# sotelo/parrot

Hardware: AMD Instinct MI355X
Metric: acoustic feature frames/sec (train fwd+bwd+allreduce+clip/Adam) (higher is better)
Workload: dtype f32; 1 GPU; BASELINE configs[1]: 2-layer attention-GRU decoder, h=1024, batch=64 per GPU, T_enc=200, T_dec=800, fp32; cell=gru, layers=2, hidden=1024, batch_per_gpu=64, global_batch=64, T_enc=200, T_dec=800, parallelism=dp1, params=13919212

## Files before the change

### include/parrot_hip.h

```cpp
#ifndef PARROT_HIP_H
#define PARROT_HIP_H

#include <stddef.h>
#include <stdint.h>

#ifdef __cplusplus
extern "C" {
#endif

#define PARROT_ERR_BADARG 10001
#define PARROT_ERR_UNSUPPORTED 10002

#define PARROT_NORM_EPS 1e-5f
#define PARROT_MAX_LAYERS 3

const char* parrot_hip_version(void);

int parrot_profile_begin(void);
long long parrot_profile_end(double* total_us, double* flops, double* bytes);
long long parrot_profile_end2(double* total_us, double* flops, double* bytes, double* plain4);

#define PARROT_PRECISION_F32 0
#define PARROT_PRECISION_BF16 1
#define PARROT_PRECISION_BF16X3 2
int parrot_set_gemm_precision(int mode);
int parrot_get_gemm_precision(void);
int parrot_gemm(const float* A, int lda, int transA, const float* B, int ldb, int transB, float* C, int ldc,
                int M, int N, int K, const float* bias, float alpha, int accumulate, int act, int nbatch,
                long long strideA, long long strideB, long long strideC, int split_k, void* stream);

int parrot_gemm_gated(const float* A, int lda, int transA, const float* B, int ldb, int transB, float* C, int ldc,
                      int M, int N, int K, const float* gate, int ldg, void* stream);

#define PARROT_GEMM_ROUTE_STEP 0
#define PARROT_GEMM_ROUTE_F32 1
#define PARROT_GEMM_ROUTE_BF16 2
#define PARROT_GEMM_ROUTE_BF16X3 3
int parrot_gemm_route(const float* A, int lda, int transA, const float* B, int ldb, int transB, int M, int N, int K,
                      float alpha, int act, int nbatch, long long strideA, long long strideB, int split_k, int has_gate,
                      int* kernel, int* slices);

int parrot_step_launch_mode(int njobs, const int* M, const int* N, const int* K, const int* lstm_H, int* info);

int parrot_to_bf16(const float* x, void* y, long long n, void* stream);
int parrot_gemm_bf16in(const void* A, int lda, const void* B, int ldb, float* C, int ldc, int M, int N, int K,
                       int accumulate, int split_k, void* stream);
int parrot_gemm_bf16in_ex(const void* A, int lda, int transA, const void* B, int ldb, int transB, float* C, int ldc, int M,
                          int N, int K, const float* bias, int accumulate, int split_k, void* stream);

int parrot_colsum(const float* x, long long M, int N, int ld, float* out, int accumulate, void* stream);
int parrot_colsum_route(const float* x, long long M, int N, int ld, const float* out, int* info2);

int parrot_gru_step_fwd(const float* h, const float* inputs, const float* gate_inputs, const float* mask,
                        const float* Wg, const float* Wc, float* h_out, float* z, float* r, float* rh,
                        float* c, int B, int H, void* stream);

int parrot_gru_step_bwd(const float* dh_out, const float* h, const float* mask, const float* Wg,
                        const float* Wc, const float* z, const float* r, const float* c, float* dh,
                        float* d_inputs, float* d_gate_inputs, int B, int H, void* stream);

typedef struct ParrotGruSeqDesc {
    int T, B, H, nchain, use_graph, reserved;
    int reverse[4];
    const float* Wg[4];
    const float* Wc[4];
    const float* inputs[4];
    const float* gate_inputs[4];
    const float* mask;
    float* h[4];
    float* z[4]; float* r[4]; float* rh[4]; float* c[4];
    float* dh[4];
    float* dG[4];
    float* dC[4];
// ... 317 lines not shown
```

### parrot_amd/_lib.py

```python
from __future__ import annotations

import ctypes as C
import os

from .utils import env_str

_HERE = os.path.dirname(os.path.abspath(__file__))
LIB_PATH = os.path.join(_HERE, "libparrot_hip.so")

MAX_LAYERS = 3

c_float_p = C.c_void_p


class HipLibraryMissing(RuntimeError):
    pass


class HipCallError(RuntimeError):
    pass


class GruSeqDesc(C.Structure):
    _fields_ = [
# ... 119 lines not shown
        ("eou_extra", C.c_int), ("reserved9", C.c_int),
        ("Wrh_t", C.c_void_p), ("rh_const", C.c_void_p), ("rh_cols", C.c_int), ("reserved10", C.c_int),
        ("Wc_t16", C.c_void_p * MAX_LAYERS),
    ]


class SampleRnnGenDesc(C.Structure):
    _fields_ = ([(n, C.c_int) for n in ("B", "D", "T", "Q", "FS", "BFS", "feat_dim", "use_graph")] +
                [("temperature", C.c_float), ("reserved", C.c_int), ("seed", C.c_ulonglong)] +
                [(n, C.c_void_p) for n in (
                    "big_Win_frames", "big_Win_feats", "big_bin", "big_U", "big_bU", "big_Wg", "big_Wc",
                    "big_Wout", "big_bout", "frm_Win", "frm_bin", "frm_U", "frm_bU", "frm_Wg", "frm_Wc",
                    "frm_Wout", "frm_bout", "emb_tbl", "W2", "b2", "W3", "b3", "W4", "b4", "features",
                    "samples", "big_h", "frm_h", "xf_big", "xf_frm", "feat_cur", "gru_in", "P", "z", "r", "rh",
                    "big_out", "frame_out", "o1", "o2", "o3", "logits", "tbase")] +
                [("n_rnn", C.c_int), ("lstm", C.c_int),
                 ("big_L", (C.c_void_p * 4) * 5), ("frm_L", (C.c_void_p * 4) * 5),
                 ("big_hs", C.c_void_p * 5), ("big_cs", C.c_void_p * 5),
                 ("frm_hs", C.c_void_p * 5), ("frm_cs", C.c_void_p * 5),
                 ("gate_ws", C.c_void_p), ("layer_tmp", C.c_void_p),
                 ("persist_ws", C.c_void_p), ("persist_ws_floats", C.c_longlong)])


_vp, _i, _f, _ll, _sz = C.c_void_p, C.c_int, C.c_float, C.c_longlong, C.c_size_t
SIGNATURES = {
    "parrot_hip_version": (C.c_char_p, []),
    "parrot_profile_begin": (_i, []),
    "parrot_profile_end": (C.c_longlong, [C.POINTER(C.c_double)] * 3),
    "parrot_profile_end2": (C.c_longlong, [C.POINTER(C.c_double)] * 4),
    "parrot_gemm": (_i, [_vp, _i, _i, _vp, _i, _i, _vp, _i, _i, _i, _i, _vp, _f, _i, _i, _i, _ll, _ll, _ll, _i, _vp]),
    "parrot_gemm_gated": (_i, [_vp, _i, _i, _vp, _i, _i, _vp, _i, _i, _i, _i, _vp, _i, _vp]),
    "parrot_gemm_route": (_i, [_vp, _i, _i, _vp, _i, _i, _i, _i, _i, _f, _i, _i, _ll, _ll, _i, _i,
                               C.POINTER(C.c_int), C.POINTER(C.c_int)]),
    "parrot_step_launch_mode": (_i, [_i] + [C.POINTER(C.c_int)] * 5),
    "parrot_gather_sum_fwd": (_i, [_vp, _vp, _vp, _i, _vp, _i, _ll, _i, _i, _i, _vp]),
    "parrot_gather_sum_bwd_ws_floats": (C.c_longlong, [_ll, _i, _i, _i]),
    "parrot_gather_sum_bwd": (_i, [_vp, _i, _vp, _vp, _vp, _vp, _ll, _ll, _i, _i, _i, _i, _vp]),
    "parrot_softmax_ce_fwd": (_i, [_vp, _i, _vp, _ll, _i, _vp, _vp, _vp]),
    "parrot_softmax_ce_bwd": (_i, [_vp, _i, _vp, _vp, _vp, _ll, _i, _vp, _i, _vp]),
    "parrot_relu_gate": (_i, [_vp, _vp, _vp, _ll, _vp]),
    "parrot_gmm_cost_fwd": (_i, [_vp, _i] * 4 + [_ll, _i, _i, _f, _vp, _vp, _i, _vp, _vp]),
    "parrot_gmm_cost_bwd": (_i, [_vp, _i] * 4 + [_vp, _vp, _ll, _i, _i, _f] + [_vp, _i] * 3 + [_vp]),
    "samplernn_weightnorm_ws_floats": (_ll, [_i]),
    "samplernn_weightnorm_fold": (_i, [_vp, _i, _vp, _vp, _i, _vp, _vp, _i, _i, _vp]),
    "samplernn_weightnorm_fold_bwd": (_i, [_vp, _i, _vp, _vp, _vp, _i, _vp, _i, _vp, _vp, _i, _i, _i, _i, _vp]),
    "parrot_colsum": (_i, [_vp, _ll, _i, _i, _vp, _i, _vp]),
    "parrot_colsum_route": (_i, [_vp, _ll, _i, _i, _vp, C.POINTER(C.c_int)]),
    "parrot_gru_step_fwd": (_i, [_vp] * 11 + [_i, _i, _vp]),
    "parrot_gru_step_bwd": (_i, [_vp] * 11 + [_i, _i, _vp]),
    "parrot_label_tables_supported": (_i, [_ll, _i]),
    "parrot_label_gather": (_i, [C.POINTER(LabelTablesDesc), _vp]),
    "parrot_label_segsum_ws_floats": (C.c_longlong, [_ll, _i, _i]),
    "parrot_label_segsum": (_i, [C.POINTER(LabelTablesDesc), _vp, _ll, _vp]),
    "parrot_gru_seq_create": (_i, [C.POINTER(GruSeqDesc), C.POINTER(C.c_void_p)]),
    "parrot_gru_seq_fwd": (_i, [_vp, _vp]),
    "parrot_gru_seq_bwd": (_i, [_vp, _vp]),
    "parrot_gru_seq_destroy": (_i, [_vp]),
    "parrot_gru_seq_route": (_i, [_vp, C.POINTER(C.c_int)]),
    "parrot_gru_seq_rowwise_supported": (_i, [_i, _i, _i, _i]),
    "parrot_lstm_seq_create": (_i, [C.POINTER(LstmSeqDesc), C.POINTER(C.c_void_p)]),
    "parrot_lstm_seq_fwd": (_i, [_vp, _vp]),
    "parrot_lstm_seq_bwd": (_i, [_vp, _vp]),
    "parrot_lstm_seq_destroy": (_i, [_vp]),
    "parrot_gmm_attention_fwd": (_i, [_vp] * 10 + [_i] * 6 + [_f] * 4 + [_vp]),
    "parrot_gmm_attention_bwd": (_i, [_vp] * 10 + [_i] * 6 + [_f, _vp]),
    "parrot_decoder_create": (_i, [C.POINTER(DecoderDesc), C.POINTER(C.c_void_p)]),
# ... 80 lines not shown
```

### parrot_amd/csrc/biggemm.h

```cpp
#pragma once
#include "common.h"

struct BgArgs {
    const float* A;
    const float* B;
    float* C;
    const float* bias;
    int M, N, K;
    long long sam, sak, sbk, sbn;
    int ldc;
    long long batchA, batchB, batchC;
    int nbatch;
    int splitk;
    float* ws;
    int accumulate;
    float alpha;
    int act;
    const float* gate;
    int ldg;
    int bf16;
};

int bg_launch(const BgArgs& a, hipStream_t stream);
void bg_tile_shape(int bf16, int& bm, int& bn);
int bg_to_bf16_launch(const float* x, void* y, long long n, hipStream_t stream);
int bg_reduce_launch(const BgArgs& a, hipStream_t stream);

struct BgPrecisionScope {
    explicit BgPrecisionScope(int bf16);
    ~BgPrecisionScope();
    int saved;
};
```

### parrot_amd/csrc/biggemm.hip

```cpp
#include "biggemm.h"

#include <atomic>

#include <hip/hip_runtime.h>
#include <stdlib.h>
#include <string.h>

namespace {

constexpr int BM = 128, BN = 128, BK = 16, PITCH = 132;

__device__ __forceinline__ void bg_tile_of_block(int bid, int tiles_m, int tiles_n, int& tm, int& tn) {
    const int nwg = tiles_m * tiles_n;
    const int q = nwg / 8, r = nwg % 8;
    const int xcd = bid % 8, idx = bid / 8;
    const int lin = (xcd < r ? xcd * (q + 1) : r * (q + 1) + (xcd - r) * q) + idx;
    constexpr int GW = 8;
    const int group = lin / (GW * tiles_m);
    const int first = group * GW;
    const int gsz = min(tiles_n - first, GW);
    const int rem = lin - group * GW * tiles_m;
    tm = rem / gsz;
    tn = first + rem % gsz;
}

template <bool XC>
__device__ __forceinline__ void bg_load8(const float* __restrict__ p, int x0, int X, int k0, int kend,
                                         long long sx, long long sk, bool vec, int t, f32x4& v) {
    v = (f32x4){0.f, 0.f, 0.f, 0.f};
    if (XC) {
        const int xq = t & 31, kr = t >> 5;
        const int k = k0 + kr, x = x0 + 4 * xq;
        if (k < kend) {
// ... 386 lines not shown
            if (n >= a.N) continue;
            const float bias = (a.bias && ks == 0) ? a.bias[n] : 0.f;
#pragma unroll
            for (int q = 0; q < 16; ++q) {
                const int m = m0 + wm * 128 + i * 32 + (q & 3) + 8 * (q >> 2) + 4 * kk;
                if (m >= a.M) continue;
                const float v = a.alpha * acc[i][j][q];
                if (a.splitk > 1) {
                    a.ws[((long long)z * a.M + m) * a.N + n] = v;
                } else {
                    float* c = C + (long long)m * a.ldc + n;
                    *c = a.accumulate ? *c + v + bias : v + bias;
                }
            }
        }
}

constexpr int SBK = 16;
typedef __bf16 bf16x4 __attribute__((ext_vector_type(4)));

__device__ __forceinline__ void bgs_split(const f32x4& v, bf16x4& p0, bf16x4& p1, bf16x4& p2) {
    p0 = __builtin_convertvector(v, bf16x4);
    const f32x4 r1 = v - __builtin_convertvector(p0, f32x4);
    p1 = __builtin_convertvector(r1, bf16x4);
    const f32x4 r2 = r1 - __builtin_convertvector(p1, f32x4);
    p2 = __builtin_convertvector(r2, bf16x4);
}

template <bool XC>
struct BgsOperand {
    static constexpr int PK = SBK + 8;
    static constexpr int PLANE = XC ? SBK * HPITCH : 256 * PK;
    static constexpr int SZ = 3 * PLANE;
    static __device__ __forceinline__ void load(const float* __restrict__ p, long long ld, int x0, int X, int k0, int kend,
                                                bool vec, int t, f32x4 (&v)[2]) {
#pragma unroll
        for (int i = 0; i < 2; ++i) {
            const int id = t + 512 * i;
            v[i] = (f32x4){0.f, 0.f, 0.f, 0.f};
            if (XC) {
                const int k = k0 + (id >> 6), x = x0 + 4 * (id & 63);
                if (k < kend && x < X) {
                    const float* q = p + (long long)k * ld + x;
                    if (vec && x + 3 < X) v[i] = *reinterpret_cast<const f32x4*>(q);
                    else {
#pragma unroll
                        for (int u = 0; u < 4; ++u)
                            if (x + u < X) v[i][u] = q[u];
                    }
                }
            } else {
                const int x = x0 + (id >> 2), k = k0 + 4 * (id & 3);
                if (x < X && k < kend) {
                    const float* q = p + (long long)x * ld + k;
                    if (vec && k + 3 < kend) v[i] = *reinterpret_cast<const f32x4*>(q);
                    else {
#pragma unroll
                        for (int u = 0; u < 4; ++u)
                            if (k + u < kend) v[i][u] = q[u];
                    }
                }
            }
        }
    }
    static __device__ __forceinline__ void store(__bf16* __restrict__ s, int t, const f32x4 (&v)[2]) {
#pragma unroll
        for (int i = 0; i < 2; ++i) {
            const int id = t + 512 * i;
            bf16x4 p0, p1, p2;
            bgs_split(v[i], p0, p1, p2);
            __bf16* d = XC ? s + (id >> 6) * HPITCH + 4 * (id & 63) : s + (id >> 2) * PK + 4 * (id & 3);
            *reinterpret_cast<bf16x4*>(d) = p0;
            *reinterpret_cast<bf16x4*>(d + PLANE) = p1;
            *reinterpret_cast<bf16x4*>(d + 2 * PLANE) = p2;
        }
    }
    static __device__ __forceinline__ bf16x8 frag(const __bf16* __restrict__ img, int xb, int kk, int li) {
        if (XC) {
            typedef short s16x4 __attribute__((ext_vector_type(4)));
            typedef short s16x8 __attribute__((ext_vector_type(8)));
            typedef __attribute__((address_space(3))) s16x4* lds4;
            const int q = (li >> 2) & 3, xg = xb + (li & 16) + 4 * (li & 3);
            const __bf16* p = img + (8 * kk + q) * HPITCH + xg;
            const s16x4 lo = __builtin_amdgcn_ds_read_tr16_b64_v4i16((lds4)(p));
            const s16x4 hi = __builtin_amdgcn_ds_read_tr16_b64_v4i16((lds4)(p + 4 * HPITCH));
            const s16x8 v = {lo[0], lo[1], lo[2], lo[3], hi[0], hi[1], hi[2], hi[3]};
            return __builtin_bit_cast(bf16x8, v);
        } else {
            return *reinterpret_cast<const bf16x8*>(img + (xb + li) * PK + 8 * kk);
        }
    }
};

template <bool AXC, bool BXC>
__global__ __launch_bounds__(512) void bgs_kernel(const BgArgs a, int vecA, int vecB, int tiles_m, int tiles_n, int zmap) {
    typedef BgsOperand<AXC> OA;
    typedef BgsOperand<BXC> OB;
    extern __shared__ __attribute__((aligned(16))) __bf16 bgs_smem[];
    __bf16* As = bgs_smem;
    __bf16* Bs = bgs_smem + 2 * OA::SZ;
    int tm, tn, z;
    if (zmap) {
        const int tiles = tiles_m * tiles_n, idx = blockIdx.x >> 3;
        z = 8 * (idx / tiles) + (blockIdx.x & 7);
        const int tl = idx % tiles;
        tm = tl / tiles_n;
        tn = tl % tiles_n;
    } else {
        bg_tile_of_block(blockIdx.x, tiles_m, tiles_n, tm, tn);
        z = blockIdx.y;
    }
    const int m0 = tm * HBMT, n0 = tn * HBNT;
    const int batch = z / a.splitk, ks = z % a.splitk;
    int kchunk = (a.K + a.splitk - 1) / a.splitk;
    kchunk = (kchunk + SBK - 1) / SBK * SBK;
    const int kbeg = ks * kchunk;
    const int kend = min(a.K, kbeg + kchunk);
    const float* A = a.A + (long long)batch * a.batchA;
    const float* B = a.B + (long long)batch * a.batchB;
    float* C = a.C + (long long)batch * a.batchC;
    const long long lda = AXC ? a.sak : a.sam, ldb = BXC ? a.sbk : a.sbn;
    const int t = threadIdx.x, lane = t & 63, wave = t >> 6;
    const int wm = wave >> 2, wn = wave & 3;
    const int kk = lane >> 5, li = lane & 31;
    f32x16 acc[4][2];
#pragma unroll
    for (int i = 0; i < 4; ++i)
#pragma unroll
        for (int j = 0; j < 2; ++j)
#pragma unroll
            for (int q = 0; q < 16; ++q) acc[i][j][q] = 0.f;
    f32x4 ra[2], rb[2];
    const int nk = (kend - kbeg + SBK - 1) / SBK;
    if (nk > 0) {
        OA::load(A, lda, m0, a.M, kbeg, kend, vecA, t, ra);
        OB::load(B, ldb, n0, a.N, kbeg, kend, vecB, t, rb);
        OA::store(As, t, ra);
        OB::store(Bs, t, rb);
        if (nk > 1) {
            OA::load(A, lda, m0, a.M, kbeg + SBK, kend, vecA, t, ra);
            OB::load(B, ldb, n0, a.N, kbeg + SBK, kend, vecB, t, rb);
        }
    }
    __syncthreads();
    const bool early = wave >= 4;
    for (int kt = 0; kt < nk; ++kt) {
        const int cur = kt & 1;
        const __bf16* as = As + cur * OA::SZ;
        const __bf16* bs = Bs + cur * OB::SZ;
        if (early && kt + 1 < nk) {
            OA::store(As + (cur ^ 1) * OA::SZ, t, ra);
            OB::store(Bs + (cur ^ 1) * OB::SZ, t, rb);
            if (kt + 2 < nk) {
                OA::load(A, lda, m0, a.M, kbeg + (kt + 2) * SBK, kend, vecA, t, ra);
                OB::load(B, ldb, n0, a.N, kbeg + (kt + 2) * SBK, kend, vecB, t, rb);
            }
        }
        bf16x8 fb[2][3];
#pragma unroll
        for (int j = 0; j < 2; ++j)
#pragma unroll
            for (int p = 0; p < 3; ++p) fb[j][p] = OB::frag(bs + p * OB::PLANE, wn * 64 + 32 * j, kk, li);
#pragma unroll
        for (int i = 0; i < 4; ++i) {
            bf16x8 fa[3];
#pragma unroll
            for (int p = 0; p < 3; ++p) fa[p] = OA::frag(as + p * OA::PLANE, wm * 128 + 32 * i, kk, li);
#define BGS_MM(pa, pb)                                                                                    \
    acc[i][0] = __builtin_amdgcn_mfma_f32_32x32x16_bf16(fa[pa], fb[0][pb], acc[i][0], 0, 0, 0);          \
    acc[i][1] = __builtin_amdgcn_mfma_f32_32x32x16_bf16(fa[pa], fb[1][pb], acc[i][1], 0, 0, 0)
            BGS_MM(2, 0);
            BGS_MM(0, 2);
            BGS_MM(1, 1);
            BGS_MM(1, 0);
            BGS_MM(0, 1);
            BGS_MM(0, 0);
#undef BGS_MM
        }
        if (!early && kt + 1 < nk) {
            OA::store(As + (cur ^ 1) * OA::SZ, t, ra);
            OB::store(Bs + (cur ^ 1) * OB::SZ, t, rb);
            if (kt + 2 < nk) {
                OA::load(A, lda, m0, a.M, kbeg + (kt + 2) * SBK, kend, vecA, t, ra);
                OB::load(B, ldb, n0, a.N, kbeg + (kt + 2) * SBK, kend, vecB, t, rb);
            }
        }
        __syncthreads();
    }
#pragma unroll
    for (int i = 0; i < 4; ++i)
#pragma unroll
        for (int j = 0; j < 2; ++j) {
            const int n = n0 + wn * 64 + j * 32 + li;
            if (n >= a.N) continue;
            const float bias = (a.bias && ks == 0) ? a.bias[n] : 0.f;
#pragma unroll
            for (int q = 0; q < 16; ++q) {
                const int m = m0 + wm * 128 + i * 32 + (q & 3) + 8 * (q >> 2) + 4 * kk;
                if (m >= a.M) continue;
                const float v = a.alpha * acc[i][j][q];
                if (a.splitk > 1) {
                    a.ws[((long long)z * a.M + m) * a.N + n] = v;
                } else {
                    float* c = C + (long long)m * a.ldc + n;
                    float r = a.accumulate ? *c + v + bias : v + bias;
                    if (a.act == 1) r = fmaxf(r, 0.f);
                    if (a.gate && !(a.gate[(long long)m * a.ldg + n] > 0.f)) r = 0.f;
                    *c = r;
                }
            }
        }
}

__global__ __launch_bounds__(256) void bg_to_bf16_kernel(const float* __restrict__ x, __bf16* __restrict__ y, long long n8) {
    for (long long i = (long long)blockIdx.x * 256 + threadIdx.x; i < n8; i += (long long)gridDim.x * 256) {
        const f32x4 lo = *reinterpret_cast<const f32x4*>(x + 8 * i);
        const f32x4 hi = *reinterpret_cast<const f32x4*>(x + 8 * i + 4);
        *reinterpret_cast<bf16x8*>(y + 8 * i) = ph_bf16x8(lo, hi);
    }
}

__global__ __launch_bounds__(256) void bg_reduce_kernel(const BgArgs a) {
    const long long mn = (long long)a.M * a.N;
    const long long total = mn * a.nbatch;
    for (long long i = (long long)blockIdx.x * 256 + threadIdx.x; i < total; i += (long long)gridDim.x * 256) {
        const int batch = (int)(i / mn);
        const long long r = i % mn;
        const int m = (int)(r / a.N), n = (int)(r % a.N);
        float* c = a.C + (long long)batch * a.batchC + (long long)m * a.ldc + n;
        float v = a.accumulate ? *c : 0.f;
        if (a.bias) v += a.bias[n];
        const float* w = a.ws + ((long long)batch * a.splitk) * mn + r;
        int ks = 0;
        for (; ks + 8 <= a.splitk; ks += 8) {
            float p[8];
#pragma unroll
            for (int q = 0; q < 8; ++q) p[q] = w[(long long)(ks + q) * mn];
#pragma unroll
            for (int q = 0; q < 8; ++q) v += p[q];
        }
        for (; ks < a.splitk; ++ks) v += w[(long long)ks * mn];
        if (a.gate && !(a.gate[(long long)m * a.ldg + n] > 0.f)) v = 0.f;
        *c = v;
    }
}

}

int bg_reduce_launch(const BgArgs& a, hipStream_t stream) {
    const long long total = (long long)a.M * a.N * a.nbatch;
    int blocks = (int)((total + 255) / 256);
    if (blocks > 4096) blocks = 4096;
    hipLaunchKernelGGL(bg_reduce_kernel, dim3(blocks), dim3(256), 0, stream, a);
    return (int)hipGetLastError();
}

void bg_tile_shape(int bf16, int& bm, int& bn) {
    bm = bn = 128;
    if (bf16 == 2 || bf16 == 3) { bm = HBMT; bn = HBNT; return; }
}

template <typename K>
static void bg_big_lds_once(K kern, bool& done) {
    if (!done) {
        (void)hipFuncSetAttribute((const void*)kern, hipFuncAttributeMaxDynamicSharedMemorySize, 160 * 1024);
        done = true;
    }
}

template <int BKT, bool AX, bool BX>
static void bgh_go(const BgArgs& a, dim3 grid, int tm, int tn, hipStream_t stream) {
    static bool done = false;
    bg_big_lds_once(bgh_kernel<BKT, AX, BX>, done);
    const size_t lds = (size_t)4 * (BghOperand<BKT, AX>::SZ + BghOperand<BKT, BX>::SZ);
    hipLaunchKernelGGL((bgh_kernel<BKT, AX, BX>), grid, dim3(512), lds, stream, a, tm, tn);
}

template <bool AX, bool BX>
static void bgs_go(const BgArgs& a, dim3 grid, int vecA, int vecB, int tm, int tn, int zmap, hipStream_t stream) {
    static bool done = false;
    bg_big_lds_once(bgs_kernel<AX, BX>, done);
    const size_t lds = (size_t)4 * (BgsOperand<AX>::SZ + BgsOperand<BX>::SZ);
    hipLaunchKernelGGL((bgs_kernel<AX, BX>), grid, dim3(512), lds, stream, a, vecA, vecB, tm, tn, zmap);
}

int bg_to_bf16_launch(const float* x, void* y, long long n, hipStream_t stream) {
    if (n <= 0) return 0;
    if ((n & 7) || ((uintptr_t)x & 15) || ((uintptr_t)y & 15)) return PH_ERR_BADARG;
    const long long n8 = n / 8;
    int blocks = (int)((n8 + 255) / 256);
    if (blocks > 8192) blocks = 8192;
    hipLaunchKernelGGL(bg_to_bf16_kernel, dim3(blocks), dim3(256), 0, stream, x, reinterpret_cast<__bf16*>(y), n8);
    return (int)hipGetLastError();
}

int bg_launch(const BgArgs& a, hipStream_t stream) {
    const size_t pad = 0;
    if (a.M <= 0 || a.N <= 0 || a.K < 0 || a.nbatch < 1 || a.splitk < 1 || (a.splitk > 1 && !a.ws)) return PH_ERR_BADARG;
    const bool axc = (a.sam == 1), bxc = (a.sbn == 1);
    if (!axc && a.sak != 1) return PH_ERR_BADARG;
    if (!bxc && a.sbk != 1) return PH_ERR_BADARG;
    auto al = [](const float* p, long long stride, long long batch) {
        return (((uintptr_t)p & 15) == 0) && (stride % 4 == 0) && (batch % 4 == 0);
    };
    const int vecA = axc ? al(a.A, a.sak, a.batchA) : al(a.A, a.sam, a.batchA);
    const int vecB = bxc ? al(a.B, a.sbk, a.batchB) : al(a.B, a.sbn, a.batchB);
    const int tiles_m = ceil_div(a.M, BM), tiles_n = ceil_div(a.N, BN);
    dim3 grid(tiles_m * tiles_n, a.nbatch * a.splitk);
    if (a.bf16 == 2) {
        if (a.act || a.gate || ((uintptr_t)a.A & 15) || ((uintptr_t)a.B & 15) || (a.batchA & 7) || (a.batchB & 7))
            return PH_ERR_UNSUPPORTED;
        if (axc ? ((a.M & 7) || (a.sak & 7)) : ((a.K & 7) || (a.sam & 7))) return PH_ERR_UNSUPPORTED;
        if (bxc ? ((a.N & 7) || (a.sbk & 7)) : ((a.K & 7) || (a.sbn & 7))) return PH_ERR_UNSUPPORTED;
        const int tm = ceil_div(a.M, HBMT), tn = ceil_div(a.N, HBNT);
        const int bkt = (axc && bxc) ? 32 : 64;
        const dim3 g2(tm * tn, a.nbatch * a.splitk);
        if (bkt == 64) {
            if (axc && bxc) bgh_go<64, true, true>(a, g2, tm, tn, stream);
            else if (axc) bgh_go<64, true, false>(a, g2, tm, tn, stream);
            else if (bxc) bgh_go<64, false, true>(a, g2, tm, tn, stream);
            else bgh_go<64, false, false>(a, g2, tm, tn, stream);
        } else {
            bgh_go<32, true, true>(a, g2, tm, tn, stream);
        }
        return (int)hipGetLastError();
    }
    if (a.bf16 == 3) {
        if (a.act > 1) return PH_ERR_UNSUPPORTED;
        const int tm = ceil_div(a.M, HBMT), tn = ceil_div(a.N, HBNT);
        const int Z = a.nbatch * a.splitk;
        const int zmap = (Z % 8 == 0) ? 1 : 0;
        const dim3 g = zmap ? dim3(tm * tn * Z) : dim3(tm * tn, Z);
        if (axc && bxc) bgs_go<true, true>(a, g, vecA, vecB, tm, tn, zmap, stream);
        else if (axc) bgs_go<true, false>(a, g, vecA, vecB, tm, tn, zmap, stream);
        else if (bxc) bgs_go<false, true>(a, g, vecA, vecB, tm, tn, zmap, stream);
        else bgs_go<false, false>(a, g, vecA, vecB, tm, tn, zmap, stream);
        return (int)hipGetLastError();
    }
    if (a.bf16) {
        dim3 b8(512);
        if (axc && bxc) hipLaunchKernelGGL((bg_kernel_bf16<true, true>), grid, b8, pad, stream, a, vecA, vecB, tiles_m, tiles_n);
        else if (axc && !bxc) hipLaunchKernelGGL((bg_kernel_bf16<true, false>), grid, b8, pad, stream, a, vecA, vecB, tiles_m, tiles_n);
        else if (!axc && bxc) hipLaunchKernelGGL((bg_kernel_bf16<false, true>), grid, b8, pad, stream, a, vecA, vecB, tiles_m, tiles_n);
        else hipLaunchKernelGGL((bg_kernel_bf16<false, false>), grid, b8, pad, stream, a, vecA, vecB, tiles_m, tiles_n);
        return (int)hipGetLastError();
    }
    const dim3 b8(512);
    if (axc && bxc) hipLaunchKernelGGL((bg_kernel8<true, true>), grid, b8, pad, stream, a, vecA, vecB, tiles_m, tiles_n);
    else if (axc && !bxc) hipLaunchKernelGGL((bg_kernel8<true, false>), grid, b8, pad, stream, a, vecA, vecB, tiles_m, tiles_n);
    else if (!axc && bxc) hipLaunchKernelGGL((bg_kernel8<false, true>), grid, b8, pad, stream, a, vecA, vecB, tiles_m, tiles_n);
    else hipLaunchKernelGGL((bg_kernel8<false, false>), grid, b8, pad, stream, a, vecA, vecB, tiles_m, tiles_n);
    return (int)hipGetLastError();
}
```

### parrot_amd/csrc/capi.hip

```cpp
#include "../../include/parrot_hip.h"
#include "attention.h"
#include "biggemm.h"
#include "elementwise.h"
#include "quantize.h"
#include "skinny.h"
#include "switches.h"

#include <math.h>
#include <stdlib.h>
#include <string.h>

#include <atomic>

static int gemm_target_wgs() {
    return 1024;
}

static int gemm_default_mode() {
    const char* e = env_str("PARROT_GEMM_PRECISION");
    if (e && (!strcmp(e, "f32") || !strcmp(e, "0"))) return PARROT_PRECISION_F32;
    if (e && (!strcmp(e, "bf16") || !strcmp(e, "1"))) return PARROT_PRECISION_BF16;
    return PARROT_PRECISION_BF16X3;
}
static std::atomic<int> g_gemm_bf16{gemm_default_mode()};
// ... 139 lines not shown
    return bg_run(a, split_k, st);
}

int parrot_gemm(const float* A, int lda, int transA, const float* B, int ldb, int transB, float* C, int ldc,
                int M, int N, int K, const float* bias, float alpha, int accumulate, int act, int nbatch,
                long long strideA, long long strideB, long long strideC, int split_k, void* stream) { PH_ENTRY();
    return gemm_impl(A, lda, transA, B, ldb, transB, C, ldc, M, N, K, bias, alpha, accumulate, act, nbatch, strideA, strideB,
                     strideC, split_k, nullptr, 0, stream);
}

int parrot_gemm_gated(const float* A, int lda, int transA, const float* B, int ldb, int transB, float* C, int ldc,
                      int M, int N, int K, const float* gate, int ldg, void* stream) { PH_ENTRY();
    if (!gate) return PARROT_ERR_BADARG;
    return gemm_impl(A, lda, transA, B, ldb, transB, C, ldc, M, N, K, nullptr, 1.0f, 0, 0, 1, 0, 0, 0, 0, gate, ldg, stream);
}

int parrot_gemm_route(const float* A, int lda, int transA, const float* B, int ldb, int transB, int M, int N, int K,
                      float alpha, int act, int nbatch, long long strideA, long long strideB, int split_k, int has_gate,
                      int* kernel, int* slices) {
    if (!A || !B || !kernel || !slices || M < 1 || N < 1 || K < 1 || nbatch < 1) return PARROT_ERR_BADARG;
    if (has_gate && nbatch != 1) return PARROT_ERR_BADARG;
    const int route = gemm_pick_kernel(A, lda, transA, B, ldb, transB, M, N, K, alpha, act, nbatch, strideA, strideB, split_k,
                                       has_gate != 0, gemm_mode_in_force());
    int split = 1;
    if (route != PARROT_GEMM_ROUTE_STEP) {
        split = split_k > 0 ? split_k : bg_auto_split(gemm_route_bf16(route), M, N, K, act, nbatch);
        if (split > 1 && act != 0) return PARROT_ERR_BADARG;
    }
    *kernel = route;
    *slices = split;
    return 0;
}

int parrot_step_launch_mode(int njobs, const int* M, const int* N, const int* K, const int* lstm_H, int* info) {
    if (!M || !N || !K || !info || njobs < 1 || njobs > SK_MAXJOB) return PARROT_ERR_BADARG;
    SkJob jobs[SK_MAXJOB];
    for (int q = 0; q < njobs; ++q) {
        if (M[q] < 1 || N[q] < 1 || K[q] < 1) return PARROT_ERR_BADARG;
        SkJob& j = jobs[q];
        sk_job_init(j);
        const float* aligned_base = reinterpret_cast<const float*>(uintptr_t(4096));
        j.nseg = 1;
        j.seg[0] = sk_seg(aligned_base, (K[q] + 3) & ~3, aligned_base, (N[q] + 3) & ~3, K[q], 0);
        j.M = M[q]; j.N = N[q];
        j.H = lstm_H && lstm_H[q] > 0 ? lstm_H[q] : N[q];
        j.epi = lstm_H && lstm_H[q] > 0 ? SK_EPI_LSTM : SK_EPI_LINEAR;
    }
    SkLaunch Lin, L;
    const int rc = sk_make_launch(Lin, jobs, njobs);
    if (rc) return rc;
    dim3 grid;
    size_t lds;
    int mbnb;
    sk_prepare(Lin, L, grid, lds, mbnb);
    info[0] = L.zmode; info[1] = mbnb; info[2] = (int)grid.x; info[3] = (int)grid.y; info[4] = (int)grid.z;
    for (int q = 0; q < njobs; ++q) info[5 + q] = L.tile_end[q];
    return 0;
}

int parrot_to_bf16(const float* x, void* y, long long n, void* stream) { PH_ENTRY();
    if (!x || !y || n < 0) return PARROT_ERR_BADARG;
    return bg_to_bf16_launch(x, y, n, (hipStream_t)stream);
}

int parrot_gemm_bf16in_ex(const void* A, int lda, int transA, const void* B, int ldb, int transB, float* C, int ldc, int M,
                          int N, int K, const float* bias, int accumulate, int split_k, void* stream) { PH_ENTRY();
// ... 173 lines not shown
```

### parrot_amd/csrc/switches.h

```cpp
#pragma once
#include <stdlib.h>

static inline int env_int(const char* name, int dflt) {
    const char* e = getenv(name);
    return e ? atoi(e) : dflt;
}
static inline bool env_set(const char* name) { return getenv(name) != nullptr; }
static inline const char* env_str(const char* name) { return getenv(name); }

static inline int sw_att_dense() { return env_int("PARROT_ATT_DENSE", 0); }
static inline int sw_pm_dataflow(int dflt) { return env_int("PARROT_PM_DATAFLOW", dflt); }
static inline int sw_rg_waves() { return env_int("PARROT_RG_WAVES", 8); }
static inline int sw_wk() { return env_int("PARROT_WK", 1); }
static inline bool sw_pm_dump_plan() { return env_set("PARROT_PM_DUMP_PLAN"); }
```

### parrot_amd/ops.py

```python
from __future__ import annotations

import torch

from . import _lib
from .utils import env_int, env_str

ACT_NONE, ACT_RELU, ACT_TANH, ACT_SIGMOID = 0, 1, 2, 3


def _stream() -> int:
    return torch.cuda.current_stream().cuda_stream


def _chk(t: torch.Tensor, name: str, dtype=torch.float32):
    if not isinstance(t, torch.Tensor) or not t.is_cuda:
        raise _lib.HipCallError(
            f"{name}: the parrot_amd product path needs a GPU tensor (got {type(t).__name__}"
            f"{'' if not isinstance(t, torch.Tensor) else ' on ' + str(t.device)}); there is no CPU fallback")
    if t.dtype != dtype:
        raise TypeError(f"{name}: expected {dtype}, got {t.dtype}")


def ptr(t, name="tensor", dtype=torch.float32) -> int:
    if t is None:
# ... 19 lines not shown


def gemm(a: torch.Tensor, b: torch.Tensor, bias=None, out=None, accumulate=False, act=ACT_NONE,
         alpha=1.0, split_k=0) -> torch.Tensor:
    if accumulate and int(act) != ACT_NONE:
        raise ValueError("gemm: accumulate together with an activation is not defined")
    pa, M, K, lda, ta = _mat(a, "a")
    pb, K2, N, ldb, tb = _mat(b, "b")
    if K != K2:
        raise ValueError(f"gemm: inner dimensions differ ({K} vs {K2})")
    if out is None:
        if accumulate:
            out = torch.zeros((M, N), device=a.device, dtype=torch.float32)
        else:
            out = torch.empty((M, N), device=a.device, dtype=torch.float32)
    _chk(out, "out")
    if out.shape != (M, N) or out.stride(1) != 1:
        raise ValueError("gemm: bad output tensor")
    if M == 0 or N == 0:
        return out
    if K == 0:
        if not accumulate:
            out.zero_()
        return out
    _lib.call("parrot_gemm", pa, lda, ta, pb, ldb, tb, out.data_ptr(), out.stride(0), M, N, K,
              ptr(bias, "bias"), float(alpha), int(bool(accumulate)), int(act), 1, 0, 0, 0, int(split_k),
              _stream())
    return out


ROUTE_STEP, ROUTE_F32, ROUTE_BF16, ROUTE_BF16X3 = 0, 1, 2, 3


def gemm_route(a: torch.Tensor, b: torch.Tensor, bias=None, out=None, accumulate=False, act=ACT_NONE, alpha=1.0,
               split_k=0, gate=None, nbatch=None, transA=False, transB=False):
    import ctypes as C
    if nbatch is not None:
        _chk(a, "a"); _chk(b, "b")
        if a.shape[0] != nbatch or b.shape[0] != nbatch:
            raise ValueError("gemm_route: nbatch does not match the operands")
        M, K = (a.shape[2], a.shape[1]) if transA else (a.shape[1], a.shape[2])
        N = b.shape[1] if transB else b.shape[2]
        args = (a.data_ptr(), a.stride(1), int(transA), b.data_ptr(), b.stride(1), int(transB), M, N, K, 1.0, 0,
                int(nbatch), a.stride(0), b.stride(0), 1, 0)
    else:
        pa, M, K, lda, ta = _mat(a, "a")
        pb, K2, N, ldb, tb = _mat(b, "b")
        if K != K2:
            raise ValueError(f"gemm_route: inner dimensions differ ({K} vs {K2})")
        if gate is not None:
            args = (pa, lda, ta, pb, ldb, tb, M, N, K, 1.0, 0, 1, 0, 0, 0, 1)
        else:
            args = (pa, lda, ta, pb, ldb, tb, M, N, K, float(alpha), int(act), 1, 0, 0, int(split_k), 0)
    kernel, slices = C.c_int(-1), C.c_int(-1)
    _lib.call("parrot_gemm_route", *args, C.byref(kernel), C.byref(slices))
    return kernel.value, slices.value


def to_bf16(x: torch.Tensor, out=None) -> torch.Tensor:
    _chk(x, "x")
    if not x.is_contiguous() or x.numel() % 8:
        raise ValueError("to_bf16: contiguous tensor with a multiple of 8 elements expected")
    if out is None:
        out = torch.empty(x.shape, device=x.device, dtype=torch.bfloat16)
    if out.dtype != torch.bfloat16 or out.numel() != x.numel() or not out.is_contiguous() or not out.is_cuda:
        raise ValueError("to_bf16: bad output tensor")
    _lib.call("parrot_to_bf16", x.data_ptr(), out.data_ptr(), x.numel(), _stream())
    return out


def gemm_bf16in(a_t: torch.Tensor, b: torch.Tensor, out: torch.Tensor, accumulate=False, split_k=0) -> torch.Tensor:
    for x_, n_ in ((a_t, "a_t"), (b, "b")):
        if not (x_.is_cuda and x_.dtype == torch.bfloat16 and x_.dim() == 2 and x_.stride(1) == 1):
            raise ValueError(f"gemm_bf16in: {n_} must be a 2-d bf16 GPU tensor with unit inner stride")
    _chk(out, "out")
    K, M = a_t.shape
    K2, N = b.shape
    if K != K2 or out.shape != (M, N) or out.stride(1) != 1:
        raise ValueError("gemm_bf16in: shapes do not match")
    _lib.call("parrot_gemm_bf16in", a_t.data_ptr(), a_t.stride(0), b.data_ptr(), b.stride(0), out.data_ptr(),
              out.stride(0), M, N, K, int(bool(accumulate)), int(split_k), _stream())
    return out


def gemm16(a: torch.Tensor, b: torch.Tensor, out=None, bias=None, accumulate=False, split_k=0) -> torch.Tensor:
    pa, M, K, lda, ta = _mat16(a, "a")
    pb, K2, N, ldb, tb = _mat16(b, "b")
    if K != K2:
        raise ValueError(f"gemm16: inner dimensions differ ({K} vs {K2})")
# ... 756 lines not shown
```

Baseline: 916,700 frames/s.

## Add unguarded interior bf16x3 GEMM body and 16x16x32 MFMA variant with transposed LDS reads

```diff
diff --git a/include/parrot_hip.h b/include/parrot_hip.h
--- a/include/parrot_hip.h
+++ b/include/parrot_hip.h
@@ -39,6 +39,10 @@
 int parrot_gemm_route(const float* A, int lda, int transA, const float* B, int ldb, int transB, int M, int N, int K,
                       float alpha, int act, int nbatch, long long strideA, long long strideB, int split_k, int has_gate,
                       int* kernel, int* slices);
+
+int parrot_gemm_split_variant(const float* A, int lda, int transA, const float* B, int ldb, int transB, int M, int N, int K,
+                              float alpha, int act, int nbatch, long long strideA, long long strideB, int split_k,
+                              int has_gate, int* variant, int* mfma);
 
 int parrot_step_launch_mode(int njobs, const int* M, const int* N, const int* K, const int* lstm_H, int* info);
 
diff --git a/parrot_amd/_lib.py b/parrot_amd/_lib.py
--- a/parrot_amd/_lib.py
+++ b/parrot_amd/_lib.py
@@ -175,6 +175,8 @@
     "parrot_gemm_gated": (_i, [_vp, _i, _i, _vp, _i, _i, _vp, _i, _i, _i, _i, _vp, _i, _vp]),
     "parrot_gemm_route": (_i, [_vp, _i, _i, _vp, _i, _i, _i, _i, _i, _f, _i, _i, _ll, _ll, _i, _i,
                                C.POINTER(C.c_int), C.POINTER(C.c_int)]),
+    "parrot_gemm_split_variant": (_i, [_vp, _i, _i, _vp, _i, _i, _i, _i, _i, _f, _i, _i, _ll, _ll, _i, _i,
+                                       C.POINTER(C.c_int), C.POINTER(C.c_int)]),
     "parrot_step_launch_mode": (_i, [_i] + [C.POINTER(C.c_int)] * 5),
     "parrot_gather_sum_fwd": (_i, [_vp, _vp, _vp, _i, _vp, _i, _ll, _i, _i, _i, _vp]),
     "parrot_gather_sum_bwd_ws_floats": (C.c_longlong, [_ll, _i, _i, _i]),
diff --git a/parrot_amd/csrc/biggemm.h b/parrot_amd/csrc/biggemm.h
--- a/parrot_amd/csrc/biggemm.h
+++ b/parrot_amd/csrc/biggemm.h
@@ -23,6 +23,7 @@
 
 int bg_launch(const BgArgs& a, hipStream_t stream);
 void bg_tile_shape(int bf16, int& bm, int& bn);
+void bg_split_variant(const BgArgs& a, int& full, int& mfma);
 int bg_to_bf16_launch(const float* x, void* y, long long n, hipStream_t stream);
 int bg_reduce_launch(const BgArgs& a, hipStream_t stream);
 
diff --git a/parrot_amd/csrc/biggemm.hip b/parrot_amd/csrc/biggemm.hip
--- a/parrot_amd/csrc/biggemm.hip
+++ b/parrot_amd/csrc/biggemm.hip
@@ -1,4 +1,5 @@
 #include "biggemm.h"
+#include "switches.h"
 
 #include <atomic>
 
@@ -451,11 +452,17 @@
     static constexpr int PK = SBK + 8;
     static constexpr int PLANE = XC ? SBK * HPITCH : 256 * PK;
     static constexpr int SZ = 3 * PLANE;
+    template <bool FULL>
     static __device__ __forceinline__ void load(const float* __restrict__ p, long long ld, int x0, int X, int k0, int kend,
                                                 bool vec, int t, f32x4 (&v)[2]) {
 #pragma unroll
         for (int i = 0; i < 2; ++i) {
             const int id = t + 512 * i;
+            if (FULL) {
+                static_assert(XC || !FULL, "the interior body is built for x-contiguous operands only");
+                v[i] = *reinterpret_cast<const f32x4*>(p + (long long)(k0 + (id >> 6)) * ld + x0 + 4 * (id & 63));
+                continue;
+            }
             v[i] = (f32x4){0.f, 0.f, 0.f, 0.f};
             if (XC) {
                 const int k = k0 + (id >> 6), x = x0 + 4 * (id & 63);
@@ -509,9 +516,42 @@
             return *reinterpret_cast<const bf16x8*>(img + (xb + li) * PK + 8 * kk);
         }
     }
+    static __device__ __forceinline__ bf16x8 frag16(const __bf16* __restrict__ img, int xb, int lane, int lo, int hi) {
+        static_assert(XC, "the term-paired body is built for x-contiguous operands only");
+        typedef short s16x4 __attribute__((ext_vector_type(4)));
+        typedef short s16x8 __attribute__((ext_vector_type(8)));
+        typedef __attribute__((address_space(3))) s16x4* lds4;
+        const int g = lane >> 4, i16 = lane & 15, odd = g & 1;
+        const __bf16* p = img + (g >> 1 ? hi : lo) * PLANE + (12 * odd + (i16 >> 2)) * HPITCH + xb + 4 * (i16 & 3);
+        const s16x4 v0 = __builtin_amdgcn_ds_read_tr16_b64_v4i16((lds4)(p));
+        const s16x4 v1 = __builtin_amdgcn_ds_read_tr16_b64_v4i16((lds4)(p + (odd ? -4 : 4) * HPITCH));
+        const s16x8 v = {v0[0], v0[1], v0[2], v0[3], v1[0], v1[1], v1[2], v1[3]};
+        return __builtin_bit_cast(bf16x8, v);
+    }
 };
 
-template <bool AXC, bool BXC>
+#ifdef BGS_TIMERS
+__constant__ unsigned long long* bgs_timer_buf = nullptr;
+__device__ __forceinline__ unsigned long long bgs_now() {
+    unsigned long long t;
+    __builtin_amdgcn_sched_barrier(0);
+    asm volatile("s_memtime %0\n\ts_waitcnt lgkmcnt(0)" : "=s"(t) : : "memory");
+    __builtin_amdgcn_sched_barrier(0);
+    return t;
+}
+__device__ __forceinline__ unsigned long long bgs_wall() {
+    unsigned long long t;
+    __builtin_amdgcn_sched_barrier(0);
+    asm volatile("s_memrealtime %0\n\ts_waitcnt lgkmcnt(0)" : "=s"(t) : : "memory");
+    __builtin_amdgcn_sched_barrier(0);
+    return t;
+}
+#define BGS_STAMP(kt, i) do { if ((kt) == kmid) ts[i] = bgs_now(); } while (0)
+#else
+#define BGS_STAMP(kt, i) do { } while (0)
+#endif
+
+template <bool AXC, bool BXC, bool FULL, int MM>
 __global__ __launch_bounds__(512) void bgs_kernel(const BgArgs a, int vecA, int vecB, int tiles_m, int tiles_n, int zmap) {
     typedef BgsOperand<AXC> OA;
     typedef BgsOperand<BXC> OB;
@@ -543,92 +583,178 @@
     const int wm = wave >> 2, wn = wave & 3;
     const int kk = lane >> 5, li = lane & 31;
     f32x16 acc[4][2];
-#pragma unroll
-    for (int i = 0; i < 4; ++i)
-#pragma unroll
-        for (int j = 0; j < 2; ++j)
-#pragma unroll
-            for (int q = 0; q < 16; ++q) acc[i][j][q] = 0.f;
+    f32x4 acc16[8][4];
+    if (MM == 0) {
+#pragma unroll
+        for (int i = 0; i < 4; ++i)
+#pragma unroll
+            for (int j = 0; j < 2; ++j)
+#pragma unroll
+                for (int q = 0; q < 16; ++q) acc[i][j][q] = 0.f;
+    } else {
+#pragma unroll
+        for (int i = 0; i < 8; ++i)
+#pragma unroll
+            for (int j = 0; j < 4; ++j) acc16[i][j] = (f32x4){0.f, 0.f, 0.f, 0.f};
+    }
     f32x4 ra[2], rb[2];
     const int nk = (kend - kbeg + SBK - 1) / SBK;
-    if (nk > 0) {
-        OA::load(A, lda, m0, a.M, kbeg, kend, vecA, t, ra);
-        OB::load(B, ldb, n0, a.N, kbeg, kend, vecB, t, rb);
+#ifdef BGS_TIMERS
+    const int kmid = nk / 2;
+    unsigned long long ts[8] = {0, 0, 0, 0, 0, 0, 0, 0};
+#endif
+    if (FULL || nk > 0) {
+        OA::template load<FULL>(A, lda, m0, a.M, kbeg, kend, vecA, t, ra);
+        OB::template load<FULL>(B, ldb, n0, a.N, kbeg, kend, vecB, t, rb);
         OA::store(As, t, ra);
         OB::store(Bs, t, rb);
         if (nk > 1) {
-            OA::load(A, lda, m0, a.M, kbeg + SBK, kend, vecA, t, ra);
-            OB::load(B, ldb, n0, a.N, kbeg + SBK, kend, vecB, t, rb);
+            OA::template load<FULL>(A, lda, m0, a.M, kbeg + SBK, kend, vecA, t, ra);
+            OB::template load<FULL>(B, ldb, n0, a.N, kbeg + SBK, kend, vecB, t, rb);
         }
     }
     __syncthreads();
+#ifdef BGS_TIMERS
+    const unsigned long long loop_c0 = bgs_now(), loop_w0 = bgs_wall();
+#endif
     const bool early = wave >= 4;
-    for (int kt = 0; kt < nk; ++kt) {
+    auto tile = [&](const int kt, const bool st, const bool ld) __attribute__((always_inline)) {
         const int cur = kt & 1;
         const __bf16* as = As + cur * OA::SZ;
         const __bf16* bs = Bs + cur * OB::SZ;
-        if (early && kt + 1 < nk) {
+        BGS_STAMP(kt, 0);
+        if (early && st) {
             OA::store(As + (cur ^ 1) * OA::SZ, t, ra);
             OB::store(Bs + (cur ^ 1) * OB::SZ, t, rb);
-            if (kt + 2 < nk) {
-                OA::load(A, lda, m0, a.M, kbeg + (kt + 2) * SBK, kend, vecA, t, ra);
-                OB::load(B, ldb, n0, a.N, kbeg + (kt + 2) * SBK, kend, vecB, t, rb);
-            }
-        }
-        bf16x8 fb[2][3];
-#pragma unroll
-        for (int j = 0; j < 2; ++j)
-#pragma unroll
-            for (int p = 0; p < 3; ++p) fb[j][p] = OB::frag(bs + p * OB::PLANE, wn * 64 + 32 * j, kk, li);
-#pragma unroll
-        for (int i = 0; i < 4; ++i) {
-            bf16x8 fa[3];
-#pragma unroll
-            for (int p = 0; p < 3; ++p) fa[p] = OA::frag(as + p * OA::PLANE, wm * 128 + 32 * i, kk, li);
+            BGS_STAMP(kt, 1);
+            if (ld) {
+                OA::template load<FULL>(A, lda, m0, a.M, kbeg + (kt + 2) * SBK, kend, vecA, t, ra);
+                OB::template load<FULL>(B, ldb, n0, a.N, kbeg + (kt + 2) * SBK, kend, vecB, t, rb);
+            }
+            BGS_STAMP(kt, 2);
+        }
+        BGS_STAMP(kt, 3);
+        if constexpr (MM == 0) {
+            bf16x8 fb[2][3];
+#pragma unroll
+            for (int j = 0; j < 2; ++j)
+#pragma unroll
+                for (int p = 0; p < 3; ++p) fb[j][p] = OB::frag(bs + p * OB::PLANE, wn * 64 + 32 * j, kk, li);
+#pragma unroll
+            for (int i = 0; i < 4; ++i) {
+                bf16x8 fa[3];
+#pragma unroll
+                for (int p = 0; p < 3; ++p) fa[p] = OA::frag(as + p * OA::PLANE, wm * 128 + 32 * i, kk, li);
+                if (i == 0) BGS_STAMP(kt, 6);
 #define BGS_MM(pa, pb)                                                                                    \
     acc[i][0] = __builtin_amdgcn_mfma_f32_32x32x16_bf16(fa[pa], fb[0][pb], acc[i][0], 0, 0, 0);          \
     acc[i][1] = __builtin_amdgcn_mfma_f32_32x32x16_bf16(fa[pa], fb[1][pb], acc[i][1], 0, 0, 0)
-            BGS_MM(2, 0);
-            BGS_MM(0, 2);
-            BGS_MM(1, 1);
-            BGS_MM(1, 0);
-            BGS_MM(0, 1);
-            BGS_MM(0, 0);
+                BGS_MM(2, 0);
+                BGS_MM(0, 2);
+                BGS_MM(1, 1);
+                BGS_MM(1, 0);
+                BGS_MM(0, 1);
+                BGS_MM(0, 0);
 #undef BGS_MM
-        }
-        if (!early && kt + 1 < nk) {
+            }
+        } else {
+            bf16x8 fb[4][2];
+#pragma unroll
+            for (int j = 0; j < 4; ++j) {
+                fb[j][0] = OB::frag16(bs, wn * 64 + 16 * j, lane, 0, 1);
+                fb[j][1] = OB::frag16(bs, wn * 64 + 16 * j, lane, 0, 2);
+            }
+#pragma unroll
+            for (int i = 0; i < 8; ++i) {
+                const bf16x8 f21 = OA::frag16(as, wm * 128 + 16 * i, lane, 1, 0);
+                const bf16x8 f31 = OA::frag16(as, wm * 128 + 16 * i, lane, 2, 0);
+                const bf16x8 f12 = OA::frag16(as, wm * 128 + 16 * i, lane, 0, 1);
+                if (i == 0) BGS_STAMP(kt, 6);
+#pragma unroll
+                for (int j = 0; j < 4; ++j) acc16[i][j] = __builtin_amdgcn_mfma_f32_16x16x32_bf16(f21, fb[j][1], acc16[i][j], 0, 0, 0);
+#pragma unroll
+                for (int j = 0; j < 4; ++j) acc16[i][j] = __builtin_amdgcn_mfma_f32_16x16x32_bf16(f31, fb[j][0], acc16[i][j], 0, 0, 0);
+#pragma unroll
+                for (int j = 0; j < 4; ++j) acc16[i][j] = __builtin_amdgcn_mfma_f32_16x16x32_bf16(f12, fb[j][0], acc16[i][j], 0, 0, 0);
+            }
+        }
+        BGS_STAMP(kt, 4);
+        if (!early && st) {
             OA::store(As + (cur ^ 1) * OA::SZ, t, ra);
             OB::store(Bs + (cur ^ 1) * OB::SZ, t, rb);
-            if (kt + 2 < nk) {
-                OA::load(A, lda, m0, a.M, kbeg + (kt + 2) * SBK, kend, vecA, t, ra);
-                OB::load(B, ldb, n0, a.N, kbeg + (kt + 2) * SBK, kend, vecB, t, rb);
-            }
-        }
+            BGS_STAMP(kt, 1);
+            if (ld) {
+                OA::template load<FULL>(A, lda, m0, a.M, kbeg + (kt + 2) * SBK, kend, vecA, t, ra);
+                OB::template load<FULL>(B, ldb, n0, a.N, kbeg + (kt + 2) * SBK, kend, vecB, t, rb);
+            }
+            BGS_STAMP(kt, 2);
+        }
+        BGS_STAMP(kt, 5);
         __syncthreads();
-    }
-#pragma unroll
-    for (int i = 0; i < 4; ++i)
-#pragma unroll
-        for (int j = 0; j < 2; ++j) {
-            const int n = n0 + wn * 64 + j * 32 + li;
-            if (n >= a.N) continue;
-            const float bias = (a.bias && ks == 0) ? a.bias[n] : 0.f;
-#pragma unroll
-            for (int q = 0; q < 16; ++q) {
-                const int m = m0 + wm * 128 + i * 32 + (q & 3) + 8 * (q >> 2) + 4 * kk;
-                if (m >= a.M) continue;
-                const float v = a.alpha * acc[i][j][q];
-                if (a.splitk > 1) {
-                    a.ws[((long long)z * a.M + m) * a.N + n] = v;
-                } else {
-                    float* c = C + (long long)m * a.ldc + n;
-                    float r = a.accumulate ? *c + v + bias : v + bias;
-                    if (a.act == 1) r = fmaxf(r, 0.f);
-                    if (a.gate && !(a.gate[(long long)m * a.ldg + n] > 0.f)) r = 0.f;
-                    *c = r;
+    };
+    if (FULL) {
+        int kt = 0;
+        for (; kt + 2 < nk; ++kt) tile(kt, true, true);
+        if (kt + 1 < nk) tile(kt++, true, false);
+        tile(kt, false, false);
+    } else {
+        for (int kt = 0; kt < nk; ++kt) tile(kt, kt + 1 < nk, kt + 2 < nk);
+    }
+#ifdef BGS_TIMERS
+    {
+        const unsigned long long loop_c1 = bgs_now(), loop_w1 = bgs_wall();
+        if (bgs_timer_buf && lane == 0 && (wave & 3) == 0) {
+            unsigned long long* tb = bgs_timer_buf + (size_t)blockIdx.x * 32;
+            if (wave == 0) {
+                tb[0] = loop_c0; tb[1] = loop_w0; tb[2] = loop_c1; tb[3] = loop_w1; tb[4] = (unsigned long long)nk;
+            }
+            for (int s_ = 0; s_ < 8; ++s_) tb[(wave == 0 ? 8 : 16) + s_] = ts[s_];
+        }
+    }
+#endif
+    auto put = [&](const int m, const int n, const float acc_, const float bias) __attribute__((always_inline)) {
+        const float v = a.alpha * acc_;
+        if (a.splitk > 1) {
+            a.ws[((long long)z * a.M + m) * a.N + n] = v;
+        } else {
+            float* c = C + (long long)m * a.ldc + n;
+            float r = a.accumulate ? *c + v + bias : v + bias;
+            if (a.act == 1) r = fmaxf(r, 0.f);
+            if (a.gate && !(a.gate[(long long)m * a.ldg + n] > 0.f)) r = 0.f;
+            *c = r;
+        }
+    };
+    if (MM == 0) {
+#pragma unroll
+        for (int i = 0; i < 4; ++i)
+#pragma unroll
+            for (int j = 0; j < 2; ++j) {
+                const int n = n0 + wn * 64 + j * 32 + li;
+                if (!FULL && n >= a.N) continue;
+                const float bias = (a.bias && ks == 0) ? a.bias[n] : 0.f;
+#pragma unroll
+                for (int q = 0; q < 16; ++q) {
+                    const int m = m0 + wm * 128 + i * 32 + (q & 3) + 8 * (q >> 2) + 4 * kk;
+                    if (!FULL && m >= a.M) continue;
+                    put(m, n, acc[i][j][q], bias);
                 }
             }
-        }
+    } else {
+#pragma unroll
+        for (int i = 0; i < 8; ++i)
+#pragma unroll
+            for (int j = 0; j < 4; ++j) {
+                const int n = n0 + wn * 64 + j * 16 + (lane & 15);
+                if (!FULL && n >= a.N) continue;
+                const float bias = (a.bias && ks == 0) ? a.bias[n] : 0.f;
+#pragma unroll
+                for (int q = 0; q < 4; ++q) {
+                    const int m = m0 + wm * 128 + i * 16 + 4 * (lane >> 4) + q;
+                    if (!FULL && m >= a.M) continue;
+                    put(m, n, acc16[i][j][q], bias);
+                }
+            }
+    }
 }
 
 __global__ __launch_bounds__(256) void bg_to_bf16_kernel(const float* __restrict__ x, __bf16* __restrict__ y, long long n8) {
@@ -695,12 +821,34 @@
     hipLaunchKernelGGL((bgh_kernel<BKT, AX, BX>), grid, dim3(512), lds, stream, a, tm, tn);
 }
 
-template <bool AX, bool BX>
-static void bgs_go(const BgArgs& a, dim3 grid, int vecA, int vecB, int tm, int tn, int zmap, hipStream_t stream) {
+template <bool AX, bool BX, bool FULL, int MM>
+static void bgs_go2(const BgArgs& a, dim3 grid, int vecA, int vecB, int tm, int tn, int zmap, hipStream_t stream) {
     static bool done = false;
-    bg_big_lds_once(bgs_kernel<AX, BX>, done);
+    bg_big_lds_once(bgs_kernel<AX, BX, FULL, MM>, done);
     const size_t lds = (size_t)4 * (BgsOperand<AX>::SZ + BgsOperand<BX>::SZ);
-    hipLaunchKernelGGL((bgs_kernel<AX, BX>), grid, dim3(512), lds, stream, a, vecA, vecB, tm, tn, zmap);
+    hipLaunchKernelGGL((bgs_kernel<AX, BX, FULL, MM>), grid, dim3(512), lds, stream, a, vecA, vecB, tm, tn, zmap);
+}
+
+static void bgs_go_tn(const BgArgs& a, dim3 grid, int vecA, int vecB, int tm, int tn, int zmap, int full, int mm,
+                      hipStream_t stream) {
+    if (full && mm) bgs_go2<true, true, true, 1>(a, grid, vecA, vecB, tm, tn, zmap, stream);
+    else if (full) bgs_go2<true, true, true, 0>(a, grid, vecA, vecB, tm, tn, zmap, stream);
+    else if (mm) bgs_go2<true, true, false, 1>(a, grid, vecA, vecB, tm, tn, zmap, stream);
+    else bgs_go2<true, true, false, 0>(a, grid, vecA, vecB, tm, tn, zmap, stream);
+}
+
+static bool bg_vec_ok(const float* p, long long stride, long long batch) {
+    return (((uintptr_t)p & 15) == 0) && (stride % 4 == 0) && (batch % 4 == 0);
+}
+
+void bg_split_variant(const BgArgs& a, int& full, int& mfma) {
+    const bool axc = (a.sam == 1), bxc = (a.sbn == 1);
+    const bool vecA = axc ? bg_vec_ok(a.A, a.sak, a.batchA) : bg_vec_ok(a.A, a.sam, a.batchA);
+    const bool vecB = bxc ? bg_vec_ok(a.B, a.sbk, a.batchB) : bg_vec_ok(a.B, a.sbn, a.batchB);
+    const bool ktiles = a.splitk >= 1 && a.K % a.splitk == 0 && (a.K / a.splitk) % SBK == 0 && a.K > 0;
+    const bool tn = axc && bxc;
+    full = tn && sw_bgs_full() != 0 && a.M % HBMT == 0 && a.N % HBNT == 0 && vecA && vecB && ktiles;
+    mfma = tn && sw_bgs_mfma() != 0;
 }
 
 int bg_to_bf16_launch(const float* x, void* y, long long n, hipStream_t stream) {
@@ -719,11 +867,8 @@
     const bool axc = (a.sam == 1), bxc = (a.sbn == 1);
     if (!axc && a.sak != 1) return PH_ERR_BADARG;
     if (!bxc && a.sbk != 1) return PH_ERR_BADARG;
-    auto al = [](const float* p, long long stride, long long batch) {
-        return (((uintptr_t)p & 15) == 0) && (stride % 4 == 0) && (batch % 4 == 0);
-    };
-    const int vecA = axc ? al(a.A, a.sak, a.batchA) : al(a.A, a.sam, a.batchA);
-    const int vecB = bxc ? al(a.B, a.sbk, a.batchB) : al(a.B, a.sbn, a.batchB);
+    const int vecA = axc ? bg_vec_ok(a.A, a.sak, a.batchA) : bg_vec_ok(a.A, a.sam, a.batchA);
+    const int vecB = bxc ? bg_vec_ok(a.B, a.sbk, a.batchB) : bg_vec_ok(a.B, a.sbn, a.batchB);
     const int tiles_m = ceil_div(a.M, BM), tiles_n = ceil_div(a.N, BN);
     dim3 grid(tiles_m * tiles_n, a.nbatch * a.splitk);
     if (a.bf16 == 2) {
@@ -750,10 +895,12 @@
         const int Z = a.nbatch * a.splitk;
         const int zmap = (Z % 8 == 0) ? 1 : 0;
         const dim3 g = zmap ? dim3(tm * tn * Z) : dim3(tm * tn, Z);
-        if (axc && bxc) bgs_go<true, true>(a, g, vecA, vecB, tm, tn, zmap, stream);
-        else if (axc) bgs_go<true, false>(a, g, vecA, vecB, tm, tn, zmap, stream);
-        else if (bxc) bgs_go<false, true>(a, g, vecA, vecB, tm, tn, zmap, stream);
-        else bgs_go<false, false>(a, g, vecA, vecB, tm, tn, zmap, stream);
+        int full, mm;
+        bg_split_variant(a, full, mm);
+        if (axc && bxc) bgs_go_tn(a, g, vecA, vecB, tm, tn, zmap, full, mm, stream);
+        else if (axc) bgs_go2<true, false, false, 0>(a, g, vecA, vecB, tm, tn, zmap, stream);
+        else if (bxc) bgs_go2<false, true, false, 0>(a, g, vecA, vecB, tm, tn, zmap, stream);
+        else bgs_go2<false, false, false, 0>(a, g, vecA, vecB, tm, tn, zmap, stream);
         return (int)hipGetLastError();
     }
     if (a.bf16) {
diff --git a/parrot_amd/csrc/capi.hip b/parrot_amd/csrc/capi.hip
--- a/parrot_amd/csrc/capi.hip
+++ b/parrot_amd/csrc/capi.hip
@@ -195,6 +195,30 @@
     return 0;
 }
 
+int parrot_gemm_split_variant(const float* A, int lda, int transA, const float* B, int ldb, int transB, int M, int N, int K,
+                              float alpha, int act, int nbatch, long long strideA, long long strideB, int split_k,
+                              int has_gate, int* variant, int* mfma) {
+    if (!variant || !mfma) return PARROT_ERR_BADARG;
+    int route, split;
+    const int rc = parrot_gemm_route(A, lda, transA, B, ldb, transB, M, N, K, alpha, act, nbatch, strideA, strideB, split_k,
+                                     has_gate, &route, &split);
+    if (rc) return rc;
+    *variant = 0;
+    *mfma = -1;
+    if (route != PARROT_GEMM_ROUTE_BF16X3) return 0;
+    BgArgs a = {};
+    a.A = A; a.B = B;
+    a.M = M; a.N = N; a.K = K;
+    a.sam = transA ? 1 : lda; a.sak = transA ? lda : 1;
+    a.sbk = transB ? 1 : ldb; a.sbn = transB ? ldb : 1;
+    a.batchA = strideA; a.batchB = strideB;
+    a.nbatch = nbatch;
+    a.splitk = split;
+    a.bf16 = 3;
+    bg_split_variant(a, *variant, *mfma);
+    return 0;
+}
+
 int parrot_step_launch_mode(int njobs, const int* M, const int* N, const int* K, const int* lstm_H, int* info) {
     if (!M || !N || !K || !info || njobs < 1 || njobs > SK_MAXJOB) return PARROT_ERR_BADARG;
     SkJob jobs[SK_MAXJOB];
diff --git a/parrot_amd/csrc/switches.h b/parrot_amd/csrc/switches.h
--- a/parrot_amd/csrc/switches.h
+++ b/parrot_amd/csrc/switches.h
@@ -13,3 +13,5 @@
 static inline int sw_rg_waves() { return env_int("PARROT_RG_WAVES", 8); }
 static inline int sw_wk() { return env_int("PARROT_WK", 1); }
 static inline bool sw_pm_dump_plan() { return env_set("PARROT_PM_DUMP_PLAN"); }
+static inline int sw_bgs_full() { return env_int("PARROT_BGS_FULL", 1); }
+static inline int sw_bgs_mfma() { return env_int("PARROT_BGS_MFMA", 1); }
diff --git a/parrot_amd/ops.py b/parrot_amd/ops.py
--- a/parrot_amd/ops.py
+++ b/parrot_amd/ops.py
@@ -75,9 +75,7 @@
 ROUTE_STEP, ROUTE_F32, ROUTE_BF16, ROUTE_BF16X3 = 0, 1, 2, 3
 
 
-def gemm_route(a: torch.Tensor, b: torch.Tensor, bias=None, out=None, accumulate=False, act=ACT_NONE, alpha=1.0,
-               split_k=0, gate=None, nbatch=None, transA=False, transB=False):
-    import ctypes as C
+def _route_args(a, b, act, alpha, split_k, gate, nbatch, transA, transB):
     if nbatch is not None:
         _chk(a, "a"); _chk(b, "b")
         if a.shape[0] != nbatch or b.shape[0] != nbatch:
@@ -95,9 +93,29 @@
             args = (pa, lda, ta, pb, ldb, tb, M, N, K, 1.0, 0, 1, 0, 0, 0, 1)
         else:
             args = (pa, lda, ta, pb, ldb, tb, M, N, K, float(alpha), int(act), 1, 0, 0, int(split_k), 0)
+    return args
+
+
+def gemm_route(a: torch.Tensor, b: torch.Tensor, bias=None, out=None, accumulate=False, act=ACT_NONE, alpha=1.0,
+               split_k=0, gate=None, nbatch=None, transA=False, transB=False):
+    import ctypes as C
+    args = _route_args(a, b, act, alpha, split_k, gate, nbatch, transA, transB)
     kernel, slices = C.c_int(-1), C.c_int(-1)
     _lib.call("parrot_gemm_route", *args, C.byref(kernel), C.byref(slices))
     return kernel.value, slices.value
+
+
+SPLIT_GUARDED, SPLIT_INTERIOR = 0, 1
+SPLIT_MFMA_32X32X16, SPLIT_MFMA_16X16X32 = 0, 1
+
+
+def gemm_split_variant(a: torch.Tensor, b: torch.Tensor, bias=None, out=None, accumulate=False, act=ACT_NONE, alpha=1.0,
+                       split_k=0, gate=None, nbatch=None, transA=False, transB=False):
+    import ctypes as C
+    args = _route_args(a, b, act, alpha, split_k, gate, nbatch, transA, transB)
+    variant, mfma = C.c_int(-2), C.c_int(-2)
+    _lib.call("parrot_gemm_split_variant", *args, C.byref(variant), C.byref(mfma))
+    return variant.value, mfma.value
 
 
 def to_bf16(x: torch.Tensor, out=None) -> torch.Tensor:
```

Result: no change. 923,900 frames/s, median of 6 (+0.8%).
